# fjdf/slaMEM

Hardware: AMD Instinct MI355X
Metric: MEMs/sec (and queries/sec) on 100 Mbp ref x 10 M 150 bp queries, l=20 (higher is better)
Workload: dtype u32; 1 GPU; synthetic 100000000 bp reference (splitmix64 seed 42) x 10000000 reads/GPU of 150 bp, 2% substitutions, 50% reverse-complemented, -b -l 20; ref_len=100000000, reads_total=10000000, read_len=150, min_len=20, both_strands=True, parallelism=query shards x1, one GPU, no replication

## Files before the change

slamem_amd/csrc/mem_search.hip:

```cpp
#include "common.h"
#include "prims.h"

#include <atomic>
#include <type_traits>
#include <new>
#include <stdlib.h>
#include <string.h>

namespace slamem {

struct Blk {
    uint4 a;
    uint4 b;
    uint4 c;
    uint4 d;
};

__device__ __forceinline__ uint64_t u64_of(uint32_t lo, uint32_t hi) { return ((uint64_t)hi << 32) | lo; }

__device__ __forceinline__ Blk load_blk(const FMBlock* __restrict__ fm, uint32_t bi) {
    const uint4* p = reinterpret_cast<const uint4*>(fm + bi);
    Blk k;
    k.a = p[0]; k.b = p[1]; k.c = p[2]; k.d = p[3];
    return k;
// ... 82 lines not shown
__device__ __forceinline__ int parent_from(const uint4& rt, const uint4& rb, uint32_t& top, uint32_t& bot) {
    uint32_t a = rt.x, b = rb.z;
    uint32_t d = a > b ? a : b;
    if (d == 0u) return -1;
    if (a == d) top = rt.y;
    if (b == d) bot = rb.w - 1u;
    return (int)(d - 1u);
}

__device__ __forceinline__ int parent(const IndexView& ix, uint32_t& top, uint32_t& bot) {
    const uint4* R = reinterpret_cast<const uint4*>(ix.rec);
    uint4 rt = R[top], rb = R[bot];
    return parent_from(rt, rb, top, bot);
}

__device__ __forceinline__ uint32_t ascii_code_q(uint32_t ch) {
    uint32_t x = ch & 0xDFu;
    return x == 'A' ? 2u : x == 'C' ? 3u : x == 'G' ? 4u : x == 'T' ? 5u : 1u;
}

struct SearchArgs {
    IndexView ix;
    const uint64_t* qwords;
    const uint64_t* offsets;
    uint32_t num_queries;
    uint32_t strands;
    uint32_t min_len;
    int32_t pad0;
    uint32_t pad1;
    uint32_t pad;
    uint64_t capacity;
    unsigned long long* total;
    RawKey* raw_key;
    slamem_mem* raw_mem;
    uint32_t* block_counts;
    struct RawRow* inline_rows;
    uint64_t inline_stride;
    const struct ItemDesc* items;
    uint64_t num_items;
    uint8_t* item_attempt;
    const uint8_t* item_alive;
    const uint32_t* work_ids;
    const uint32_t* work_count;
    unsigned long long* stats;
    uint64_t query_words;
    const uint64_t* pq;
    uint64_t* pq_out;
    uint32_t implicit_items;
    uint32_t* seed_left_ids;
    unsigned int* seed_left_count;
    unsigned int* seed_long_flag;
    unsigned int* seed_wide;
    uint32_t seed_step;
    const uint64_t* item_pk;
    unsigned int* work_cursor;
    int32_t direct_min_depth;
    uint32_t use_jump;
    uint32_t pad2;
    uint32_t skip_w;
    const uint64_t* pq2;
    uint64_t* pq2_out;
    uint8_t* item_flags;
    uint32_t skip_s1;
    uint32_t pad4;
    const struct SliceState* slice_state;
    const uint32_t* item_block;
    struct OutCtx {
        struct RawRow* inline_rows;
        uint64_t inline_stride;
        RawKey* raw_key;
        slamem_mem* raw_mem;
        unsigned long long* total;
        uint64_t capacity;
        uint32_t* block_counts;
        uint8_t* item_attempt;
    } prev;
    struct DeferCtx {
        struct JobRec* queue;
        unsigned int* njobs;
        uint32_t* pool;
        unsigned int* pool_next;
        uint32_t pool_cap;
        uint32_t queue_cap;
        uint32_t epoch;
        uint32_t* raw_seg;
        uint2* list;
        unsigned int* nlist;
        uint8_t* inline_valid;
    } defer;
    const struct CarryRec* carry_in;
    const unsigned int* carry_in_count;
    struct CarryRec* carry_out;
    unsigned int* carry_out_count;
};

struct RawRow { uint32_t row, pos, len; };
constexpr uint32_t kInlineMems = 4;
constexpr uint32_t kFetch = 64;

constexpr uint32_t kSliceLen = 4096;
static_assert(kSliceLen == kSearchSliceLen, "stream.hip tells the slice count of a batch from this length");
constexpr uint32_t kWarmUp = 1024;
constexpr uint32_t kMaxAttempt = 7;
struct __attribute__((aligned(16))) ItemDesc {
    uint64_t base;
    uint32_t len;
// ... 1819 lines not shown
                const uint32_t my_wave = threadIdx.x >> 6;
                res = 0;
#pragma unroll 1
                for (uint32_t first = 0; first < 4u; first += per_part) {
                    lo = span_lo(first, per_part);
                    hi = span_hi(first, per_part);
                    if (hi <= lo) continue;
                    __syncthreads();
                    pack_span(lo, (uint32_t)(hi - lo));
                    if (my_wave >= first && my_wave < first + per_part)
                        res = prefilter_item_packed<kStats>(A, d, s_pk, s_nm, (uint32_t)(d.base - (lo << 4)), n_probe);
                }
            } else {
                res = prefilter_item<kStats>(A, d, n_probe, n_qload);
            }
        }
    } else {
        res = prefilter_item<kStats>(A, d, n_probe, n_qload);
    }
    if (live) alive[g] = res;
    if (kStats) {
        stat_flush<kStats>(A.stats + SC_PF_PROBES, n_probe);
        stat_flush<kStats>(A.stats + SC_PF_QUERY_LOADS, n_qload);
        stat_flush<kStats>(A.stats + SC_PF_ITEMS, live ? 1u : 0u);
    }
}

__global__ void __launch_bounds__(256) k_prefilter_list(SearchArgs A, const uint32_t* __restrict__ list, const uint32_t* __restrict__ list_count,
                                                        uint8_t* __restrict__ alive) {
    const uint32_t count = *list_count;
    for (uint32_t i = blockIdx.x * blockDim.x + threadIdx.x; i < count; i += gridDim.x * blockDim.x) {
        const uint32_t g = list[i];
        const ItemDesc d = item_of(A, g);
        uint32_t n_probe = 0, n_qload = 0;
        if (!prefilter_item<false>(A, d, n_probe, n_qload)) alive[g] = 0;
    }
}

#ifndef SLAMEM_SEED_READS
#define SLAMEM_SEED_READS 21
#endif
constexpr uint32_t kSeedReads = SLAMEM_SEED_READS, kSeedReadsMid = 16, kSeedReadsLong = 16;
constexpr uint32_t kSeedMaxLen = 192;
constexpr uint32_t kSeedMaxLenMid = 256;
constexpr uint32_t kSeedMaxLenLong = 384;
#ifndef SLAMEM_SEED_JOBS
#define SLAMEM_SEED_JOBS 16
#endif
constexpr uint32_t kSeedJobs = SLAMEM_SEED_JOBS;
#ifndef SLAMEM_SEED_MEMS
#define SLAMEM_SEED_MEMS 12
#endif
constexpr uint32_t kSeedMems = SLAMEM_SEED_MEMS;
constexpr uint32_t kSigLetters = 12, kSigMask = (1u << kSigLetters) - 1u, kSigKnown = 1u << 24;

template <uint32_t NW, uint32_t R>
struct SeedWave {
    static constexpr uint32_t kJobs = kSeedJobs * R * NW / 3u, kMems = kSeedMems * R * NW / 3u;
    uint64_t pl[R][2][2][NW + 1];
    uint32_t len[R];
    uint32_t nwin[R];
    union {
        uint4 raw[R * NW * 4 + 1];
        struct {
            uint32_t job_p[kJobs], job_x[kJobs];
            uint32_t mem_key[kMems], mem_ref[kMems];
            uint32_t mem_sig[kMems];
        };
    };
    uint32_t bad[R];
    uint64_t pn[R][NW + 1];
    uint32_t hasn;
    unsigned long long expl[R];
    union {
        uint16_t ring[128];
        unsigned long long smask[2 * R];
    };
    uint32_t flags;
    uint32_t pad[3];
};

__device__ __forceinline__ void wave_sync() {
    __builtin_amdgcn_fence(__ATOMIC_RELEASE, "wavefront");
    __builtin_amdgcn_wave_barrier();
    __builtin_amdgcn_fence(__ATOMIC_ACQUIRE, "wavefront");
}
__device__ __forceinline__ uint64_t funnel64(uint64_t lo, uint64_t hi, uint32_t sh) { return (lo >> sh) | ((hi << 1) << (63u - sh)); }
__device__ __forceinline__ uint64_t bits_below(int x) {
    const int c = x < 0 ? 0 : x > 64 ? 64 : x;
    return c == 0 ? 0ull : (~0ull >> (64 - c));
}
__device__ __forceinline__ uint64_t bits_range(int lo, int hi) { return bits_below(hi) & ~bits_below(lo); }
__device__ __forceinline__ uint32_t sel4(const uint4& v, uint32_t a) {
    const uint32_t lo = (a & 1u) ? v.y : v.x, hi = (a & 1u) ? v.w : v.z;
    return (a & 2u) ? hi : lo;
}
__device__ __forceinline__ uint32_t sel12(const uint4& b0, const uint4& b1, const uint4& b2, uint32_t e) {
    const uint32_t a = e & 3u, x0 = sel4(b0, a), x1 = sel4(b1, a), x2 = sel4(b2, a);
    return e < 4u ? x0 : e < 8u ? x1 : x2;
}
__device__ __forceinline__ uint32_t byte_tops(uint32_t m) {
    const uint32_t y = m >> 7;
    return (y | (y >> 7) | (y >> 14) | (y >> 21)) & 0xFu;
}

#ifndef SLAMEM_SEED_WAVES
#define SLAMEM_SEED_WAVES 1
#endif
template <bool kStats, uint32_t NW, uint32_t R>
__global__ void __launch_bounds__(256, SLAMEM_SEED_WAVES) k_seed_mems(SearchArgs A, uint8_t* __restrict__ alive) {
    constexpr uint32_t kMaxLen = 64u * NW;
    static_assert(R <= 32u && R * NW <= 128u, "a flag word holds a bit per read; the planes step runs in at most two passes");
    __shared__ SeedWave<NW, R> lds[4];
    const IndexView& ix = A.ix;
    const uint32_t lane = threadIdx.x & 63u, wv = threadIdx.x >> 6;
    SeedWave<NW, R>& S = lds[wv];
    const uint32_t strands = A.strands, k = ix.seed_k, L = A.min_len, s = L - k + 1u;
    const uint32_t kmask = (1u << k) - 1u;
    const uint64_t r0 = ((uint64_t)blockIdx.x * 4u + wv) * R;
    if (r0 >= (uint64_t)A.num_queries) return;
    const uint32_t nr = (uint64_t)A.num_queries - r0 < R ? (uint32_t)((uint64_t)A.num_queries - r0) : R;
    const unsigned long long below = (1ull << lane) - 1ull;
    const int64_t ulast = (int64_t)text_units(ix.n) - 1;
    uint32_t n_win = 0, n_cmp = 0, n_nm = 0, n_mem = 0;

    const uint64_t off = lane <= nr ? A.offsets[r0 + lane] : 0ull;
    constexpr uint32_t kRawChunks = R * NW * 4u + 1u, kSpecIters = (kRawChunks + 63u) / 64u;
#ifndef SLAMEM_SEED_NO_SPEC
    constexpr bool kSpec = kSpecIters <= 5u;
#else
    constexpr bool kSpec = false;
#endif
    uint4 sv[kSpec ? kSpecIters : 1u];
    uint64_t g0 = 0, len0 = 0;
    bool spec = false;
    if (kSpec) {
        const uint64_t o0 = A.offsets[0], o1 = A.offsets[1], o_end = A.offsets[A.num_queries];
        len0 = o1 - o0;
        g0 = o0 + r0 * len0;
        const uint64_t g1 = g0 + (uint64_t)nr * len0;
        spec = len0 != 0ull && len0 <= (uint64_t)kMaxLen && g1 <= o_end;
        const uint32_t gn = spec ? (uint32_t)(((g1 - 1u) >> 4) - (g0 >> 4) + 1u) : 0u;
        const uint4* src = reinterpret_cast<const uint4*>(A.qwords) + (g0 >> 4);
#pragma unroll
        for (uint32_t j = 0; j < kSpecIters; j++) {
            const uint32_t c = lane + 64u * j;
            sv[j] = c < gn ? src[c] : make_uint4(0, 0, 0, 0);
        }
    }
    const uint64_t offn = __shfl_down(off, 1);
    if (kSpec) spec = spec && __ballot(lane <= nr && off != g0 + (uint64_t)lane * len0) == 0ull;
    uint32_t len = 0, nwin = 0;
    bool left = false;
    if (lane < nr) {
        const uint64_t l64 = offn - off;
        if (l64 > kSliceLen) atomicOr(A.seed_long_flag, 1u);
// ... 75 lines not shown
                const uint32_t tt = B2 & ~B1, good = (B0 ^ tt) & ~((B4 ^ tt) | B3 | B7) & B6;
                bad |= ~good & M;
                const uint32_t X = ((B1 ^ B2) & M) | ((B2 & M) << 4);
                const uint32_t G = (X | (X >> 7) | (X >> 14) | (X >> 21)) & 0xFFu;
                if (t < 8u) { p0lo |= (G & 0xFu) << (4u * t); p1lo |= (G >> 4) << (4u * t); }
                else { p0hi |= (G & 0xFu) << (4u * (t - 8u)); p1hi |= (G >> 4) << (4u * (t - 8u)); }
            }
            S.pl[i][0][0][j] = u64_of(p0lo, p0hi);
            S.pl[i][0][1][j] = u64_of(p1lo, p1hi);
            uint32_t nlo = 0, nhi = 0;
            if (bad && text_pure) {
#pragma unroll
                for (uint32_t t = 0; t < 16u; t++) {
                    const uint32_t d = __builtin_amdgcn_alignbyte(w[t + 1u], w[t], sh8);
                    const uint32_t nb = nv > 4u * t ? (nv - 4u * t < 4u ? nv - 4u * t : 4u) : 0u;
                    const uint32_t M = nb >= 4u ? 0x01010101u : (0x01010101u & ((1u << (8u * nb)) - 1u));
                    const uint32_t B0 = d, B1 = d >> 1, B2 = d >> 2, B3 = d >> 3, B4 = d >> 4, B6 = d >> 6, B7 = d >> 7;
                    const uint32_t tt = B2 & ~B1, X = ~((B0 ^ tt) & ~((B4 ^ tt) | B3 | B7) & B6) & M;
                    const uint32_t G = (X | (X >> 7) | (X >> 14) | (X >> 21)) & 0xFu;
                    if (t < 8u) nlo |= G << (4u * t); else nhi |= G << (4u * (t - 8u));
                }
                S.hasn = 1u;
            } else if (bad) S.bad[i] = 1u;
            S.pn[i][j] = u64_of(nlo, nhi);
        } else if (on) {
            S.pl[i][0][0][j] = 0ull; S.pl[i][0][1][j] = 0ull; S.pn[i][j] = 0ull;
        }
        if (on && j == 0u) { S.pl[i][0][0][NW] = 0ull; S.pl[i][0][1][NW] = 0ull; S.pl[i][1][0][NW] = 0ull; S.pl[i][1][1][NW] = 0ull; S.pn[i][NW] = 0ull; }
    }
    wave_sync();
    for (uint32_t pb = 0; pb < nr * NW; pb += 64u) {
        const uint32_t pp = pb + lane, i = pp / NW, w = pp % NW;
        const bool on = pp < nr * NW;
        const uint32_t Li = __shfl(plen, (int)(on ? i : 0u));
        if (on) {
            const uint32_t sh = kMaxLen - Li, q = sh >> 6, r = sh & 63u;
#pragma unroll
            for (uint32_t pl = 0; pl < 2u; pl++) {
                const uint64_t* f = S.pl[i][0][pl];
                const uint64_t lo = w + q < NW ? __brevll(f[NW - 1u - (w + q)]) : 0ull, hi = w + q + 1u < NW ? __brevll(f[NW - 2u - (w + q)]) : 0ull;
                S.pl[i][1][pl][w] = Li ? ~funnel64(lo, hi, r) & bits_range(0, (int)Li - 64 * (int)w) : 0ull;
            }
        }
    }
    {
        const bool isbad = lane < nr && plen != 0u && S.bad[lane] != 0u;
        wflags |= (uint32_t)__ballot(isbad);
        if (isbad) nwin = 0;
        if (lane < nr) { S.len[lane] = nwin ? len : 0u; S.nwin[lane] = nwin; }
    }
    if (lane == 0u)
        for (uint32_t i = nr; i < R; i++) { S.len[i] = 0u; S.nwin[i] = 0u; }
    wave_sync();
    const uint32_t mfit = k / s > 6u ? 6u : k / s;
    const uint32_t mstep = A.seed_step ? A.seed_step : mfit >= 3u ? mfit : s <= 12u ? 2u : 1u;

    const bool wave_hasn = __builtin_amdgcn_readfirstlane((int)S.hasn) != 0;
    uint32_t lg_slots = 0;
    {
        const uint32_t nwl = lane < nr ? S.nwin[lane] : 0u;
#pragma unroll
        for (uint32_t t = 1, lg = 1; t <= 32u; t <<= 1, lg++)
            if (__ballot(nwl > t) != 0ull) lg_slots = lg;
    }
    if (lane < R) S.expl[lane] = 0ull;
    uint32_t njobs = 0, nmems = 0;

    auto search = [&](auto with_n) {
    constexpr bool hasn = decltype(with_n)::value;
    auto trip = [&](uint32_t ent, bool act, uint32_t step) {
        const uint32_t rs = ent >> 8, wi = ent & 0xFFu;
        const uint32_t Lr = act ? S.len[rs] : 0u;
        const uint32_t o = wi * s;
        uint32_t want = 0, pal = 0;
        uint4 b0 = make_uint4(0, 0, 0, 0), b1 = b0, b2 = b0, b3 = b0;
        if (hasn && act) {
            const uint64_t* PN = S.pn[rs];
            if (((uint32_t)funnel64(PN[o >> 6], PN[(o >> 6) + 1u], o & 63u) & kmask) != 0u) act = false;
        }
        if (act) {
            const uint32_t q = o >> 6, sh = o & 63u;
            const uint64_t* P0 = S.pl[rs][0][0];
            const uint64_t* P1 = S.pl[rs][0][1];
            const uint32_t f0 = (uint32_t)funnel64(P0[q], P0[q + 1u], sh) & kmask, f1 = (uint32_t)funnel64(P1[q], P1[q + 1u], sh) & kmask;
            uint32_t bucket, tagbits, orient;
            seed_place(f0, f1, k, ix.seed_log2, bucket, tagbits, orient, pal);
            want = tagbits | (orient << 7);
            const uint4* B = reinterpret_cast<const uint4*>(ix.seed + bucket);
            b0 = B[0]; b1 = B[1]; b2 = B[2]; b3 = B[3];
        }
        if (kStats) n_win += (uint32_t)__popcll(__ballot(act));
        const uint32_t wbytes = want * 0x01010101u;
        const uint32_t x0 = b3.x ^ wbytes, x1 = b3.y ^ wbytes, x2 = b3.z ^ wbytes;
        const uint32_t m0 = ~((x0 & 0x7F7F7F7Fu) + 0x7F7F7F7Fu) & 0x80808080u, m1 = ~((x1 & 0x7F7F7F7Fu) + 0x7F7F7F7Fu) & 0x80808080u,
                       m2 = ~((x2 & 0x7F7F7F7Fu) + 0x7F7F7F7Fu) & 0x80808080u;
        const uint32_t count = b3.w;
        uint32_t hits = byte_tops(m0) | (byte_tops(m1) << 4) | (byte_tops(m2) << 8);
        const uint32_t rev = byte_tops(x0 & 0x80808080u) | (byte_tops(x1 & 0x80808080u) << 4) | (byte_tops(x2 & 0x80808080u) << 8);
        hits &= count >= kSeedSlots ? 0xFFFu : (1u << count) - 1u;
        if (strands == 1u && step == 1u) hits &= ~rev;
        if (!act) hits = 0;
        const uint32_t xn = act && (count & kSeedSpilled) ? (count >> 24) & 0x1Fu : 0u, xo = (count & 0xFFFFFFu) << 2;
        if (act && count > kSeedSlots && !(count & kSeedSpilled)) {
            atomicOr(&S.flags, 1u << rs);
            if (kStats) atomicAdd(A.stats + SC_SEED_WHY + 1u, 1ull);
            hits = 0;
        }
        const bool both = pal != 0u && strands == 2u;
        if (kStats && both && hits) atomicAdd(A.stats + SC_SEED_WHY + 2u, 1ull);
        const uint32_t e1 = hits ? (uint32_t)__ffs((int)hits) - 1u : 0u;
        const uint32_t p1 = sel12(b0, b1, b2, e1);
        const uint32_t st1 = (rev >> e1) & 1u;
        const uint32_t dist = step * s;
        uint32_t pn = 0, pp1 = 0, ps1 = 0;
        if (dist <= k) {
            pp1 = __shfl_up(p1, 1);
            ps1 = __shfl_up(hits ? st1 : 2u, 1);
            const uint32_t pent = __shfl_up(act ? ent : 0xFFFFFFFFu, 1);
            pn = (lane == 0u || wi < step || pent != ent - step || ps1 == 2u) ? 0u : 1u;
        }
        const uint32_t njobs0 = njobs;
        auto push = [&](bool hv, uint32_t p, uint32_t st) {
            const uint32_t w = st ? p + dist : p - dist;
            const bool job = hv && !(pn && pp1 == w && ps1 == st);
            const unsigned long long qb = __ballot(job);
            const uint32_t at = njobs + (uint32_t)__popcll(qb & below);
            if (job && at < SeedWave<NW, R>::kJobs) {
                S.job_p[at] = p;
                S.job_x[at] = (st ? Lr - k - o : o) | (st << 15) | (rs << 16);
            }
            njobs += (uint32_t)__popcll(qb);
        };
        uint32_t rem = hits;
        for (uint32_t it = 0; __ballot(rem != 0u) != 0ull; it++) {
            const bool hv = rem != 0u;
            const uint32_t e = it == 0u ? e1 : hv ? (uint32_t)__ffs((int)rem) - 1u : 0u;
            rem &= rem - 1u;
            const uint32_t p = it == 0u ? p1 : sel12(b0, b1, b2, e);
            push(hv, p, (rev >> e) & 1u);
            if (__ballot(hv && both) != 0ull) push(hv && both, p, 1u);
        }
        for (uint32_t e0 = 0; __ballot(e0 < xn) != 0ull; e0 += 4u) {
            const bool on = e0 < xn;
            uint4 v0 = make_uint4(0, 0, 0, 0), v1 = v0;
            if (on) {
                const uint4* P = reinterpret_cast<const uint4*>(ix.spill + xo + e0);
                v0 = P[0]; v1 = P[1];
            }
#pragma unroll
            for (uint32_t q = 0; q < 4u; q++) {
                const uint32_t p = q == 0u ? v0.x : q == 1u ? v0.z : q == 2u ? v1.x : v1.z;
                const uint32_t d = ((q == 0u ? v0.y : q == 1u ? v0.w : q == 2u ? v1.y : v1.w) ^ want) & 0xFFu;
                const uint32_t st = d >> 7;
                const bool hv = on && e0 + q < xn && (d & 0x7Fu) == 0u && !(strands == 1u && st && step == 1u);
                if (__ballot(hv) == 0ull) continue;
                push(hv, p, st);
                if (__ballot(hv && both) != 0ull) push(hv && both, p, 1u);
            }
        }
        if (njobs > SeedWave<NW, R>::kJobs) {
            if (act) atomicOr(&S.flags, 1u << rs);
            if (kStats && lane == 0u) atomicAdd(A.stats + SC_SEED_WHY + 3u, 1ull);
            njobs = njobs0;
        }
    };
    auto lookups = [&](uint32_t round) {
        const uint32_t step = round == 0u ? mstep : 1u;
        uint32_t cnt = 0;
        const uint32_t per = 64u >> lg_slots, wi = lane & ((1u << lg_slots) - 1u);
        const uint32_t wmod = wi - mstep * ((wi * (65536u / mstep + 1u)) >> 16);
        for (uint32_t r = 0;; r += per) {
            if (r < nr) {
                const uint32_t rr = r + (lane >> lg_slots);
                const uint32_t nw = (rr >= nr || ((S.flags >> rr) & 1u)) ? 0u : S.nwin[rr];
                const bool pred = wi < nw && (round == 0u ? wmod == 0u : wmod != 0u && ((S.expl[rr] >> wi) & 1ull) == 0ull);
                const unsigned long long pm = __ballot(pred);
                if (pred) S.ring[cnt + (uint32_t)__popcll(pm & below)] = (uint16_t)((rr << 8) | wi);
                cnt += (uint32_t)__popcll(pm);
            }
            const bool last = r >= nr;
            if (cnt >= 64u || (last && cnt != 0u)) {
                wave_sync();
                const bool act = lane < cnt;
                const uint32_t ent = act ? S.ring[lane] : 0u;
                const uint32_t over = lane + 64u < cnt ? S.ring[lane + 64u] : 0u;
                wave_sync();
                if (lane + 64u < cnt) S.ring[lane] = (uint16_t)over;
                cnt = cnt > 64u ? cnt - 64u : 0u;
                trip(ent, act, step);
            }
            if (last) break;
        }
        wave_sync();
    };

    auto compares = [&](uint32_t round) {
        const bool mark = round == 0u && mstep > 1u;
        const uint32_t ms = mstep * s;
        const uint32_t gone = S.flags;
        for (uint32_t jb = 0; jb < njobs; jb += 64u) {
            const bool listed = jb + lane < njobs;
            const uint32_t p = listed ? S.job_p[jb + lane] : 0u, xx = listed ? S.job_x[jb + lane] : 0u;
            const uint32_t os = xx & 0x7FFFu, st = (xx >> 15) & 1u, jr = xx >> 16;
            const bool has = listed && ((gone >> jr) & 1u) == 0u;
            const uint32_t Lj = S.len[jr];
            const int64_t d = (int64_t)p - (int64_t)os;
            const int64_t u0 = d >> 6;
            const uint32_t sh = (uint32_t)(d & 63);
            bool is_mem = false;
            uint32_t key = 0, ref = 0, sig = 0;
            if (has) {
                constexpr int NU = (int)NW + 1;
                int64_t ui[NU];
#pragma unroll
                for (int i = 0; i < NU; i++) { const int64_t u = u0 + i; ui[i] = u < 0 ? 0 : u > ulast ? ulast : u; }
                const uint4* T = reinterpret_cast<const uint4*>(ix.tpl);
                uint4 tu[NU], tx[NU];
#pragma unroll
                for (int i = 0; i < NU; i++) { tu[i] = T[2 * ui[i]]; tx[i] = T[2 * ui[i] + 1]; }
                uint64_t uq[NU], nu[NU];
                uint32_t anyn = 0;
#pragma unroll
                for (int i = 0; i < NU; i++) { nu[i] = u64_of(tx[i].x, tx[i].y); uq[i] = u64_of(tx[i].z, tx[i].w); anyn |= (tx[i].x | tx[i].y); }
                if (kStats && anyn) n_nm++;
                const uint64_t* R0 = S.pl[jr][st][0];
                const uint64_t* R1 = S.pl[jr][st][1];
                uint64_t mm[NW];
#pragma unroll
                for (int w = 0; w < (int)NW; w++)
                    mm[w] = (funnel64(u64_of(tu[w].x, tu[w].y), u64_of(tu[w + 1].x, tu[w + 1].y), sh) ^ R0[w]) |
                            (funnel64(u64_of(tu[w].z, tu[w].w), u64_of(tu[w + 1].z, tu[w + 1].w), sh) ^ R1[w]) | funnel64(nu[w], nu[w + 1], sh);
                if (hasn) {
                    const uint64_t* PN = S.pn[jr];
                    if (st == 0u) {
#pragma unroll
                        for (int w = 0; w < (int)NW; w++) mm[w] |= PN[w];
                    } else {
                        const uint32_t shn = kMaxLen - Lj, qn = shn >> 6, rn = shn & 63u;
#pragma unroll
                        for (int w = 0; w < (int)NW; w++) {
                            const uint32_t x = (uint32_t)w + qn;
                            const uint64_t lo64 = x < NW ? __brevll(PN[NW - 1u - x]) : 0ull, hi64 = x + 1u < NW ? __brevll(PN[NW - 2u - x]) : 0ull;
                            mm[w] |= funnel64(lo64, hi64, rn);
                        }
                    }
                }
                const int lo = d < 0 ? (int)(-d) : 0;
                const int64_t room = (int64_t)ix.n - d;
                const int hi = room < (int64_t)Lj ? (int)room : (int)Lj;
#pragma unroll
                for (int w = 0; w < (int)NW; w++) mm[w] |= ~bits_range(lo - 64 * w, hi - 64 * w);
                uint32_t a = 0, b = kMaxLen;
                bool broken = false;
#pragma unroll
                for (int w = 0; w < (int)NW; w++) {
                    const uint64_t lw = mm[w] & bits_range(0, (int)os - 64 * w);
                    if (lw) a = 64u * w + 64u - (uint32_t)__clzll((long long)lw);
                    if (mm[w] & bits_range((int)os - 64 * w, (int)(os + k) - 64 * w)) broken = true;
                }
#pragma unroll
                for (int w = (int)NW - 1; w >= 0; w--) {
                    const uint64_t hw = mm[w] & ~bits_range(0, (int)(os + k) - 64 * w);
                    if (hw) b = 64u * w + (uint32_t)__ffsll((unsigned long long)hw) - 1u;
                }
                const uint32_t af = st ? Lj - b : a, bf = st ? Lj - a : b, of = st ? Lj - k - os : os;
                bool owner;
                if (round == 0u) owner = !(of >= ms && of - ms >= af);
                else {
                    const uint32_t oa = (af + ms - 1u) / ms * ms;
                    owner = !(mstep > 1u && oa + k <= bf) && !(of >= s && of - s >= af);
                }
                if (broken) {
                    atomicOr(&S.flags, 1u << jr);
                    if (kStats) atomicAdd(A.stats + SC_SEED_WHY + 4u, 1ull);
                }
                else if (owner && b - a >= L && (strands == 2u || st == 0u)) {
                    is_mem = true; key = (a << 16) | (b - a); ref = (uint32_t)(d + (int64_t)a);
                    if (!anyn && b + kSigLetters <= kMaxLen && d + (int64_t)b + (int64_t)kSigLetters <= (int64_t)ix.n) {
                        const uint32_t wb = b >> 6, sb = b & 63u;
                        uint64_t l0 = 0, h0 = 0, l1 = 0, h1 = 0;
#pragma unroll
                        for (int w = 0; w < (int)NW; w++) {
                            const uint64_t t0 = funnel64(u64_of(tu[w].x, tu[w].y), u64_of(tu[w + 1].x, tu[w + 1].y), sh);
                            const uint64_t t1 = funnel64(u64_of(tu[w].z, tu[w].w), u64_of(tu[w + 1].z, tu[w + 1].w), sh);
                            if ((uint32_t)w == wb) { l0 = t0; l1 = t1; }
                            if ((uint32_t)w == wb + 1u) { h0 = t0; h1 = t1; }
                        }
                        sig = kSigKnown | ((uint32_t)funnel64(l0, h0, sb) & kSigMask) | (((uint32_t)funnel64(l1, h1, sb) & kSigMask) << kSigLetters);
                    }
                }
                if (mark && !broken && bf >= af + k) {
                    uint64_t uqs[NW];
#pragma unroll
                    for (int w = 0; w < (int)NW; w++) uqs[w] = funnel64(uq[w], uq[w + 1], sh);
                    unsigned long long done = 0ull;
                    for (uint32_t wi = (af + s - 1u) / s, wl = (bf - k) / s; wi <= wl; wi++) {
                        const uint32_t x = st ? Lj - k - wi * s : wi * s;
                        uint64_t word = 0ull;
#pragma unroll
                        for (int w = 0; w < (int)NW; w++) word = (x >> 6) == (uint32_t)w ? uqs[w] : word;
                        if ((word >> (x & 63u)) & 1ull) done |= 1ull << wi;
                    }
                    if (done) atomicOr(&S.expl[jr], done);
                }
            }
            if (kStats) {
                const uint32_t nh = (uint32_t)__popcll(__ballot(has));
                n_cmp += nh;
                if (mark && lane == 0u) atomicAdd(A.stats + SC_SEED_ONCE, (unsigned long long)nh);
            }
            const unsigned long long mb = __ballot(is_mem);
            if (is_mem) {
                const uint32_t at = nmems + (uint32_t)__popcll(mb & below);
                if (at < SeedWave<NW, R>::kMems) { S.mem_key[at] = key; S.mem_ref[at] = ref; S.mem_sig[at] = sig | ((2u * jr + st) << 25); }
                else { atomicOr(&S.flags, 1u << jr); if (kStats) atomicAdd(A.stats + SC_SEED_WHY + 5u, 1ull); }
            }
            nmems += (uint32_t)__popcll(mb);
        }
        wave_sync();
    };

    for (uint32_t round = 0; round < (mstep > 1u ? 2u : 1u); round++) {
        njobs = 0;
        lookups(round);
        compares(round);
    }
    };
    if (wave_hasn) search(std::true_type{}); else search(std::false_type{});
    {
        if (nmems > SeedWave<NW, R>::kMems) nmems = SeedWave<NW, R>::kMems;

        const uint32_t g0 = (uint32_t)(r0 * strands);
        auto rank_of = [&](uint32_t mi, uint32_t key, uint32_t g, uint32_t& rank, uint32_t& cnt, bool& tie) {
            rank = 0; cnt = 0; tie = false;
            for (uint32_t t2 = 0; t2 < nmems; t2++) {
                const uint32_t kk = S.mem_key[t2], gg = S.mem_sig[t2] >> 25;
                const bool same = gg == g;
                cnt += same ? 1u : 0u;
                rank += (same && kk > key) ? 1u : 0u;
                tie = tie || (same && kk == key && t2 != mi);
            }
        };
        auto tie_rank = [&](uint32_t mi, uint32_t key, uint32_t myref, uint32_t g, uint32_t sig, uint32_t& rank) -> bool {
            const uint32_t a = key >> 16, b = a + (key & 0xFFFFu);
            bool child = false;
            for (uint32_t t2 = 0; t2 < nmems; t2++) {
                const uint32_t kk = S.mem_key[t2], a2 = kk >> 16, b2 = a2 + (kk & 0xFFFFu);
                child = child || ((S.mem_sig[t2] >> 25) == g && kk != key && a2 <= a && b2 > b);
            }
            const uint32_t jr = g >> 1, st = g & 1u;
            uint32_t qb = 0;
            if (child) qb = (uint32_t)((S.pl[jr][st][0][b >> 6] >> (b & 63u)) & 1ull) | ((uint32_t)((S.pl[jr][st][1][b >> 6] >> (b & 63u)) & 1ull) << 1);
            auto letter = [&](uint32_t sg, uint32_t t) { return ((sg >> t) & 1u) | (((sg >> (t + kSigLetters)) & 1u) << 1); };
            const bool rows = ix.prec != nullptr;
            const uint32_t my_side = child && letter(sig, 0u) > qb ? 1u : 0u;
            bool bad = (sig & kSigKnown) == 0u && (child || !rows);
            for (uint32_t t2 = 0; t2 < nmems; t2++) {
                const uint32_t so = S.mem_sig[t2];
                if (t2 == mi || (so >> 25) != g || S.mem_key[t2] != key) continue;
                const bool known = (so & sig & kSigKnown) != 0u;
                if (!known && (child || !rows)) { bad = true; continue; }
                const uint32_t o_side = child && letter(so, 0u) > qb ? 1u : 0u;
                bool before;
                if (o_side != my_side) before = o_side == 0u;
                else {
                    const uint32_t x = sig ^ so, diff = known ? (x | (x >> kSigLetters)) & kSigMask : 0u;
                    bool smaller;
                    if (diff != 0u) {
                        const uint32_t t = (uint32_t)__ffs((int)diff) - 1u;
                        smaller = letter(so, t) < letter(sig, t);
                    } else if (rows) smaller = ix.prec[S.mem_ref[t2]].row < ix.prec[myref].row;
                    else { bad = true; continue; }
                    before = my_side == 0u ? smaller : !smaller;
                }
                rank += before ? 1u : 0u;
// ... 559 lines not shown
        STEP(hipMemsetAsync(d_pq, 0, 16, stream), "memset");
        A.pq = d_pq;
        A.pq_out = d_pq;
        A.item_pk = seed_path ? nullptr : d_itempk;
        static const int env_depth = [] { const char* v = getenv("SLAMEM_DIRECT_DEPTH"); return v ? atoi(v) : 0; }();
        int lg = 0;
        for (uint64_t v = idx->hdr.n; v > 1; v >>= 2) lg++;
        A.direct_min_depth = (idx->view.tgrp && depth_class((int)min_len) >= 1u) ? lg + 3 : -1;
        if (env_depth > 0 && A.direct_min_depth >= 0) A.direct_min_depth = env_depth;
        if (env_depth < 0) A.direct_min_depth = -1;
        static const bool env_jump = [] { const char* v = getenv("SLAMEM_KJUMP_USE"); return !(v && atoi(v) == 0); }();
        A.use_jump = env_jump ? 1u : 0u;
        {
            static const bool env_skip = [] { const char* v = getenv("SLAMEM_SKIP"); return v && atoi(v) != 0; }();
            const uint32_t kd = idx->view.kbits ? idx->view.kbits_k : 0u;
            A.skip_w = 0;
            if (env_skip && kd && min_len >= kd && min_len >= 9u && min_len < 0x10000u && A.direct_min_depth >= 0) {
                const uint32_t s1 = min_len - kd + 1u;
                const uint32_t nprobes = (kd - 1u + s1 - 1u) / s1 + 1u;
                if (nprobes <= 4u && depth_class((int)min_len - 1) >= 1u) {
                    A.skip_w = min_len - 1u;
                    A.skip_s1 = s1;
                    A.pq2 = reinterpret_cast<const uint64_t*>(ws + w.off_pq2);
                    A.pq2_out = reinterpret_cast<uint64_t*>(ws + w.off_pq2);
                    A.item_flags = reinterpret_cast<uint8_t*>(ws + w.off_itemflags);
                }
            }
        }
    }
    return SLAMEM_OK;
}

int SearchJob::prep(hipStream_t stream) {
    SLAMEM_HIP(hipSetDevice(idx->device));
    char* ws = static_cast<char*>(workspace_dev);
    unsigned long long* d_total = reinterpret_cast<unsigned long long*>(ws + w.off_total);
    uint32_t* d_counts = reinterpret_cast<uint32_t*>(ws + w.off_counts);
    prefiltered = false; timed_k8 = false; launched = true; seeded = false; rawkey_marked = false;
    (void)hipEventRecord(ev[0], stream);
    if (nitems && (match_type != 1 || mam_v3)) {
        static const bool use_filter = [] { const char* v = getenv("SLAMEM_KFILTER"); return !(v && atoi(v) == 0); }();
        seeded = seed_path;
        if (seeded) {
            uint8_t* d_alive = reinterpret_cast<uint8_t*>(ws + w.off_alive);
            if (mems_capacity && !A.skip_w && !want_stats && enum_chunks()) {
                STEP(hipMemsetAsync(ws + w.off_rawkey, 0xFF, mems_capacity * sizeof(RawKey), stream), "memset");
                rawkey_marked = true;
            }
            STEP(hipMemsetAsync(d_counts, 0, nitems * 4, stream), "memset");
            STEP(hipMemsetAsync(A.item_attempt, 0, nitems, stream), "memset");
            {
                const char* v = getenv("SLAMEM_SEED_STEP");
                A.seed_step = v && atoi(v) >= 1 && atoi(v) <= 6 ? (uint32_t)atoi(v) : 0u;
            }
            uint32_t* d_ids = reinterpret_cast<uint32_t*>(ws + w.off_workids);
            uint32_t* d_nwork = reinterpret_cast<uint32_t*>(d_total) + 8;
            A.seed_left_ids = d_ids;
            A.seed_left_count = d_nwork;
            A.seed_long_flag = reinterpret_cast<unsigned int*>(d_total) + 3;
            A.seed_wide = reinterpret_cast<unsigned int*>(d_total) + 4;
            seed_words_avg = query_bytes > (uint64_t)num_queries * kSeedMaxLenMid ? 6u : query_bytes > (uint64_t)num_queries * kSeedMaxLen ? 4u : 3u;
            const uint32_t hint = __atomic_load_n(&idx->seed_words_hint, __ATOMIC_RELAXED);
            seed_words = seed_words_avg > hint ? seed_words_avg : hint;
            const bool mid_reads = seed_words == 4u, long_reads = seed_words == 6u;
            const dim3 gs(grid_for((uint64_t)num_queries, 4 * (long_reads ? kSeedReadsLong : mid_reads ? kSeedReadsMid : kSeedReads)));
            if (long_reads) {
                if (want_stats) hipLaunchKernelGGL((k_seed_mems<true, 6, kSeedReadsLong>), gs, dim3(256), 0, stream, A, d_alive);
                else hipLaunchKernelGGL((k_seed_mems<false, 6, kSeedReadsLong>), gs, dim3(256), 0, stream, A, d_alive);
            } else if (mid_reads) {
                if (want_stats) hipLaunchKernelGGL((k_seed_mems<true, 4, kSeedReadsMid>), gs, dim3(256), 0, stream, A, d_alive);
                else hipLaunchKernelGGL((k_seed_mems<false, 4, kSeedReadsMid>), gs, dim3(256), 0, stream, A, d_alive);
            } else {
                if (want_stats) hipLaunchKernelGGL((k_seed_mems<true, 3, kSeedReads>), gs, dim3(256), 0, stream, A, d_alive);
                else hipLaunchKernelGGL((k_seed_mems<false, 3, kSeedReads>), gs, dim3(256), 0, stream, A, d_alive);
            }
            STEP(hipGetLastError(), "k_seed_mems");
            (void)hipEventRecord(ev[3], stream);
            prefiltered = true;
            A.item_alive = d_alive;
            A.work_ids = d_ids;
            A.work_count = d_nwork;
            if (use_filter && idx->view.kfilter && min_len >= idx->view.kfilter_k) {
                hipLaunchKernelGGL(k_prefilter_list, dim3(512), dim3(256), 0, stream, A, (const uint32_t*)d_ids, (const uint32_t*)d_nwork, d_alive);
                STEP(hipGetLastError(), "k_prefilter_list");
            }
        } else if (use_filter && idx->view.kfilter && min_len >= idx->view.kfilter_k) {
            uint8_t* d_alive = reinterpret_cast<uint8_t*>(ws + w.off_alive);
            if (want_stats) hipLaunchKernelGGL(k_prefilter<true>, dim3(grid_for(nitems)), dim3(256), 0, stream, A, d_alive);
            else hipLaunchKernelGGL(k_prefilter<false>, dim3(grid_for(nitems)), dim3(256), 0, stream, A, d_alive);
            STEP(hipGetLastError(), "k_prefilter");
            (void)hipEventRecord(ev[3], stream);
            prefiltered = true;
            A.item_alive = d_alive;
            STEP(hipMemsetAsync(d_counts, 0, nitems * 4, stream), "memset");
            STEP(hipMemsetAsync(A.item_attempt, 0, nitems, stream), "memset");
            uint32_t* d_ids = reinterpret_cast<uint32_t*>(ws + w.off_workids);
            uint32_t* d_nwork = reinterpret_cast<uint32_t*>(d_total) + 8;
            size_t need2 = w.select_bytes;
            STEP(select_indices_u32(ws + w.off_select, need2, d_alive, d_ids, d_nwork, nitems, stream), "select");
            A.work_ids = d_ids;
            A.work_count = d_nwork;
        }
        if (A.item_flags) STEP(hipMemsetAsync(A.item_flags, 0, nitems, stream), "memset");
        if (nitems != num_blocks) {
            static const uint32_t env_warm = [] { const char* v = getenv("SLAMEM_SLICE_WARMUP"); return v && atoi(v) > 0 ? (uint32_t)atoi(v) : kWarmUp; }();
            SliceState* d_states = reinterpret_cast<SliceState*>(ws + w.off_slicestate);
// ... 484 lines not shown
```

Measured before the change: 4.480 billion MEMs/s.

## Seed MEM search from a few sparse windows, then fill uncovered windows

Replaces the fixed-stride first round of seed lookups with a sparse first round that probes only a few evenly spaced windows per read (default 3, settable through SLAMEM_SEED_FIRST). It then marks, per query position, which k-mers are already covered by extended agreement runs, so the second round skips covered windows. A memo of the last diagonal found also suppresses duplicate jobs. The aim is fewer hash lookups and fewer reference compares per read, paid for with bit-parallel agreement masks, multi-MEM enumeration per job, and a larger shared-memory explored array, all of which add compute and register pressure.

```diff
diff --git a/slamem_amd/csrc/mem_search.hip b/slamem_amd/csrc/mem_search.hip
--- a/slamem_amd/csrc/mem_search.hip
+++ b/slamem_amd/csrc/mem_search.hip
@@ -158,6 +158,7 @@
     unsigned int* seed_long_flag;
     unsigned int* seed_wide;
     uint32_t seed_step;
+    uint32_t seed_first;
     const uint64_t* item_pk;
     unsigned int* work_cursor;
     int32_t direct_min_depth;
@@ -2083,6 +2084,11 @@
 #define SLAMEM_SEED_MEMS 12
 #endif
 constexpr uint32_t kSeedMems = SLAMEM_SEED_MEMS;
+#ifndef SLAMEM_SEED_FIRST
+#define SLAMEM_SEED_FIRST 3
+#endif
+constexpr uint32_t kSeedFirst = SLAMEM_SEED_FIRST;
+static_assert(kSeedFirst >= 1u && kSeedFirst <= 8u, "SLAMEM_SEED_FIRST: 1..8");
 constexpr uint32_t kSigLetters = 12, kSigMask = (1u << kSigLetters) - 1u, kSigKnown = 1u << 24;
 
 template <uint32_t NW, uint32_t R>
@@ -2099,10 +2105,13 @@
             uint32_t mem_sig[kMems];
         };
     };
-    uint32_t bad[R];
+    union {
+        uint32_t bad[R];
+        uint32_t adia[R];
+    };
     uint64_t pn[R][NW + 1];
     uint32_t hasn;
-    unsigned long long expl[R];
+    unsigned long long expl[R][NW];
     union {
         uint16_t ring[128];
         unsigned long long smask[2 * R];
@@ -2133,6 +2142,36 @@
 __device__ __forceinline__ uint32_t byte_tops(uint32_t m) {
     const uint32_t y = m >> 7;
     return (y | (y >> 7) | (y >> 14) | (y >> 21)) & 0xFu;
+}
+
+template <uint32_t NW>
+__device__ __forceinline__ void and_shr(uint64_t (&v)[NW], uint32_t c) {
+#pragma unroll
+    for (uint32_t w = 0; w < NW; w++) v[w] &= funnel64(v[w], w + 1u < NW ? v[w + 1u] : 0ull, c);
+}
+template <uint32_t NW>
+__device__ __forceinline__ void agree_from(const uint64_t (&mm)[NW], uint32_t k, uint64_t (&a)[NW]) {
+#pragma unroll
+    for (uint32_t w = 0; w < NW; w++) a[w] = ~mm[w];
+    uint32_t span = 1;
+    for (; 2u * span <= k; span *= 2u) and_shr<NW>(a, span);
+    if (span < k) and_shr<NW>(a, k - span);
+}
+template <uint32_t NW>
+__device__ __forceinline__ void to_forward(uint64_t (&v)[NW], uint32_t sh) {
+    uint64_t r[NW], p[NW];
+#pragma unroll
+    for (uint32_t w = 0; w < NW; w++) r[w] = __brevll(v[NW - 1u - w]);
+    const uint32_t q = sh >> 6, rr = sh & 63u;
+#pragma unroll
+    for (uint32_t i = 0; i < NW; i++) p[i] = funnel64(r[i], i + 1u < NW ? r[i + 1u] : 0ull, rr);
+#pragma unroll
+    for (uint32_t w = 0; w < NW; w++) {
+        uint64_t x = 0ull;
+#pragma unroll
+        for (uint32_t i = w; i < NW; i++) x = i == w + q ? p[i] : x;
+        v[w] = x;
+    }
 }
 
 #ifndef SLAMEM_SEED_WAVES
@@ -2314,26 +2353,45 @@
     if (lane == 0u)
         for (uint32_t i = nr; i < R; i++) { S.len[i] = 0u; S.nwin[i] = 0u; }
     wave_sync();
-    const uint32_t mfit = k / s > 6u ? 6u : k / s;
-    const uint32_t mstep = A.seed_step ? A.seed_step : mfit >= 3u ? mfit : s <= 12u ? 2u : 1u;
+    const bool sparse = A.seed_step == 0u;
+    const uint32_t mstep = sparse ? 1u : A.seed_step, nfirst = sparse ? (s <= 12u ? A.seed_first : 64u) : mstep > 1u ? 1u : 64u;
 
     const bool wave_hasn = __builtin_amdgcn_readfirstlane((int)S.hasn) != 0;
     uint32_t lg_slots = 0;
+    uint32_t nwmax = 0;
     {
         const uint32_t nwl = lane < nr ? S.nwin[lane] : 0u;
 #pragma unroll
         for (uint32_t t = 1, lg = 1; t <= 32u; t <<= 1, lg++)
             if (__ballot(nwl > t) != 0ull) lg_slots = lg;
-    }
-    if (lane < R) S.expl[lane] = 0ull;
+#pragma unroll
+        for (uint32_t bit = 64u; bit != 0u; bit >>= 1)
+            if (__ballot(nwl >= (nwmax | bit)) != 0ull) nwmax |= bit;
+    }
+    unsigned long long fwu = bits_below((int)nwmax);
+    if (mstep > 1u) {
+        unsigned long long m = 0ull;
+        for (uint32_t w = 0; w < 64u; w += mstep) m |= 1ull << w;
+        fwu &= m;
+    } else if (sparse && nwmax > nfirst) {
+        const uint32_t frcp = 65536u / (2u * nfirst) + 1u;
+        fwu = 0ull;
+        for (uint32_t j = 0; j < nfirst; j++) fwu |= 1ull << ((((2u * j + 1u) * nwmax) * frcp) >> 16);
+    }
+    auto has_b = [&](uint32_t nw) { return (bits_below((int)nw) & ~fwu) != 0ull; };
+    const bool two = __ballot(lane < nr && has_b(S.nwin[lane])) != 0ull;
+    for (uint32_t i = lane; i < R * NW; i += 64u) (&S.expl[0][0])[i] = 0ull;
+    if (lane < R) S.adia[lane] = 0xFFFFFFFFu;
+    const bool memo = (uint64_t)ix.n + 2u * kMaxLen < 0x7FFFFFFFull;
     uint32_t njobs = 0, nmems = 0;
 
     auto search = [&](auto with_n) {
     constexpr bool hasn = decltype(with_n)::value;
-    auto trip = [&](uint32_t ent, bool act, uint32_t step) {
+    auto trip = [&](uint32_t ent, bool act, uint32_t round) {
         const uint32_t rs = ent >> 8, wi = ent & 0xFFu;
         const uint32_t Lr = act ? S.len[rs] : 0u;
         const uint32_t o = wi * s;
+        const bool marks = round == 0u && act && has_b(S.nwin[rs]);
         uint32_t want = 0, pal = 0;
         uint4 b0 = make_uint4(0, 0, 0, 0), b1 = b0, b2 = b0, b3 = b0;
         if (hasn && act) {
@@ -2360,7 +2418,7 @@
         uint32_t hits = byte_tops(m0) | (byte_tops(m1) << 4) | (byte_tops(m2) << 8);
         const uint32_t rev = byte_tops(x0 & 0x80808080u) | (byte_tops(x1 & 0x80808080u) << 4) | (byte_tops(x2 & 0x80808080u) << 8);
         hits &= count >= kSeedSlots ? 0xFFFu : (1u << count) - 1u;
-        if (strands == 1u && step == 1u) hits &= ~rev;
+        if (strands == 1u && !marks) hits &= ~rev;
         if (!act) hits = 0;
         const uint32_t xn = act && (count & kSeedSpilled) ? (count >> 24) & 0x1Fu : 0u, xo = (count & 0xFFFFFFu) << 2;
         if (act && count > kSeedSlots && !(count & kSeedSpilled)) {
@@ -2373,18 +2431,15 @@
         const uint32_t e1 = hits ? (uint32_t)__ffs((int)hits) - 1u : 0u;
         const uint32_t p1 = sel12(b0, b1, b2, e1);
         const uint32_t st1 = (rev >> e1) & 1u;
-        const uint32_t dist = step * s;
-        uint32_t pn = 0, pp1 = 0, ps1 = 0;
-        if (dist <= k) {
-            pp1 = __shfl_up(p1, 1);
-            ps1 = __shfl_up(hits ? st1 : 2u, 1);
-            const uint32_t pent = __shfl_up(act ? ent : 0xFFFFFFFFu, 1);
-            pn = (lane == 0u || wi < step || pent != ent - step || ps1 == 2u) ? 0u : 1u;
-        }
+        const uint32_t ps1 = __shfl_up(hits ? st1 : 2u, 1), pp1 = __shfl_up(p1, 1), pent = __shfl_up(act ? ent : 0xFFFFFFFFu, 1);
+        const uint32_t dist1 = (wi - (pent & 0xFFu)) * s;
+        const uint32_t e1s = lane != 0u && (pent >> 8) == rs && (two || dist1 <= k) ? ps1 : 2u, e1p = ps1 ? pp1 - dist1 : pp1 + dist1;
+        const bool use_memo = round != 0u && memo && act;
+        const uint32_t adia = use_memo ? S.adia[rs] : 0xFFFFFFFFu;
         const uint32_t njobs0 = njobs;
         auto push = [&](bool hv, uint32_t p, uint32_t st) {
-            const uint32_t w = st ? p + dist : p - dist;
-            const bool job = hv && !(pn && pp1 == w && ps1 == st);
+            const uint32_t dc = (p - (st ? Lr - k - o : o) + kMaxLen) | (st << 31);
+            const bool job = hv && !(e1s == st && e1p == p) && !(use_memo && dc == adia);
             const unsigned long long qb = __ballot(job);
             const uint32_t at = njobs + (uint32_t)__popcll(qb & below);
             if (job && at < SeedWave<NW, R>::kJobs) {
@@ -2414,7 +2469,7 @@
                 const uint32_t p = q == 0u ? v0.x : q == 1u ? v0.z : q == 2u ? v1.x : v1.z;
                 const uint32_t d = ((q == 0u ? v0.y : q == 1u ? v0.w : q == 2u ? v1.y : v1.w) ^ want) & 0xFFu;
                 const uint32_t st = d >> 7;
-                const bool hv = on && e0 + q < xn && (d & 0x7Fu) == 0u && !(strands == 1u && st && step == 1u);
+                const bool hv = on && e0 + q < xn && (d & 0x7Fu) == 0u && !(strands == 1u && st && !marks);
                 if (__ballot(hv) == 0ull) continue;
                 push(hv, p, st);
                 if (__ballot(hv && both) != 0ull) push(hv && both, p, 1u);
@@ -2427,15 +2482,14 @@
         }
     };
     auto lookups = [&](uint32_t round) {
-        const uint32_t step = round == 0u ? mstep : 1u;
         uint32_t cnt = 0;
         const uint32_t per = 64u >> lg_slots, wi = lane & ((1u << lg_slots) - 1u);
-        const uint32_t wmod = wi - mstep * ((wi * (65536u / mstep + 1u)) >> 16);
         for (uint32_t r = 0;; r += per) {
             if (r < nr) {
                 const uint32_t rr = r + (lane >> lg_slots);
                 const uint32_t nw = (rr >= nr || ((S.flags >> rr) & 1u)) ? 0u : S.nwin[rr];
-                const bool pred = wi < nw && (round == 0u ? wmod == 0u : wmod != 0u && ((S.expl[rr] >> wi) & 1ull) == 0ull);
+                const bool fa = ((fwu >> wi) & 1ull) != 0ull;
+                const bool pred = wi < nw && (round == 0u ? fa : !fa && ((S.expl[rr][(wi * s) >> 6] >> ((wi * s) & 63u)) & 1ull) == 0ull);
                 const unsigned long long pm = __ballot(pred);
                 if (pred) S.ring[cnt + (uint32_t)__popcll(pm & below)] = (uint16_t)((rr << 8) | wi);
                 cnt += (uint32_t)__popcll(pm);
@@ -2449,7 +2503,7 @@
                 wave_sync();
                 if (lane + 64u < cnt) S.ring[lane] = (uint16_t)over;
                 cnt = cnt > 64u ? cnt - 64u : 0u;
-                trip(ent, act, step);
+                trip(ent, act, round);
             }
             if (last) break;
         }
@@ -2457,9 +2511,24 @@
     };
 
     auto compares = [&](uint32_t round) {
-        const bool mark = round == 0u && mstep > 1u;
-        const uint32_t ms = mstep * s;
+        const bool mark = round == 0u && two;
         const uint32_t gone = S.flags;
+        uint64_t wall[NW], fa[NW];
+        {
+            uint32_t o1 = 0;
+#pragma unroll
+            for (uint32_t w = 0; w < NW; w++) {
+                uint64_t x1 = 0ull;
+                for (; two && o1 < 64u * w + 64u; o1 += s) x1 |= 1ull << (o1 - 64u * w);
+                wall[w] = x1;
+                fa[w] = 0ull;
+            }
+            for (unsigned long long m = two ? fwu : 0ull; m != 0ull; m &= m - 1ull) {
+                const uint32_t oj = (uint32_t)(__ffsll(m) - 1) * s;
+#pragma unroll
+                for (uint32_t w = 0; w < NW; w++) fa[w] |= (oj >> 6) == w ? 1ull << (oj & 63u) : 0ull;
+            }
+        }
         for (uint32_t jb = 0; jb < njobs; jb += 64u) {
             const bool listed = jb + lane < njobs;
             const uint32_t p = listed ? S.job_p[jb + lane] : 0u, xx = listed ? S.job_x[jb + lane] : 0u;
@@ -2469,8 +2538,13 @@
             const int64_t d = (int64_t)p - (int64_t)os;
             const int64_t u0 = d >> 6;
             const uint32_t sh = (uint32_t)(d & 63);
-            bool is_mem = false;
-            uint32_t key = 0, ref = 0, sig = 0;
+            uint64_t run[NW];
+            uint64_t mm[NW];
+            uint64_t tt0[NW], tt1[NW];
+            uint32_t anyn = 0;
+            bool report = false;
+#pragma unroll
+            for (int w = 0; w < (int)NW; w++) run[w] = 0ull;
             if (has) {
                 constexpr int NU = (int)NW + 1;
                 int64_t ui[NU];
@@ -2481,17 +2555,17 @@
 #pragma unroll
                 for (int i = 0; i < NU; i++) { tu[i] = T[2 * ui[i]]; tx[i] = T[2 * ui[i] + 1]; }
                 uint64_t uq[NU], nu[NU];
-                uint32_t anyn = 0;
 #pragma unroll
                 for (int i = 0; i < NU; i++) { nu[i] = u64_of(tx[i].x, tx[i].y); uq[i] = u64_of(tx[i].z, tx[i].w); anyn |= (tx[i].x | tx[i].y); }
                 if (kStats && anyn) n_nm++;
                 const uint64_t* R0 = S.pl[jr][st][0];
                 const uint64_t* R1 = S.pl[jr][st][1];
-                uint64_t mm[NW];
-#pragma unroll
-                for (int w = 0; w < (int)NW; w++)
-                    mm[w] = (funnel64(u64_of(tu[w].x, tu[w].y), u64_of(tu[w + 1].x, tu[w + 1].y), sh) ^ R0[w]) |
-                            (funnel64(u64_of(tu[w].z, tu[w].w), u64_of(tu[w + 1].z, tu[w + 1].w), sh) ^ R1[w]) | funnel64(nu[w], nu[w + 1], sh);
+#pragma unroll
+                for (int w = 0; w < (int)NW; w++) {
+                    tt0[w] = funnel64(u64_of(tu[w].x, tu[w].y), u64_of(tu[w + 1].x, tu[w + 1].y), sh);
+                    tt1[w] = funnel64(u64_of(tu[w].z, tu[w].w), u64_of(tu[w + 1].z, tu[w + 1].w), sh);
+                    mm[w] = (tt0[w] ^ R0[w]) | (tt1[w] ^ R1[w]) | funnel64(nu[w], nu[w + 1], sh);
+                }
                 if (hasn) {
                     const uint64_t* PN = S.pn[jr];
                     if (st == 0u) {
@@ -2512,58 +2586,60 @@
                 const int hi = room < (int64_t)Lj ? (int)room : (int)Lj;
 #pragma unroll
                 for (int w = 0; w < (int)NW; w++) mm[w] |= ~bits_range(lo - 64 * w, hi - 64 * w);
-                uint32_t a = 0, b = kMaxLen;
-                bool broken = false;
-#pragma unroll
-                for (int w = 0; w < (int)NW; w++) {
-                    const uint64_t lw = mm[w] & bits_range(0, (int)os - 64 * w);
-                    if (lw) a = 64u * w + 64u - (uint32_t)__clzll((long long)lw);
-                    if (mm[w] & bits_range((int)os - 64 * w, (int)(os + k) - 64 * w)) broken = true;
-                }
-#pragma unroll
-                for (int w = (int)NW - 1; w >= 0; w--) {
-                    const uint64_t hw = mm[w] & ~bits_range(0, (int)(os + k) - 64 * w);
-                    if (hw) b = 64u * w + (uint32_t)__ffsll((unsigned long long)hw) - 1u;
-                }
-                const uint32_t af = st ? Lj - b : a, bf = st ? Lj - a : b, of = st ? Lj - k - os : os;
-                bool owner;
-                if (round == 0u) owner = !(of >= ms && of - ms >= af);
-                else {
-                    const uint32_t oa = (af + ms - 1u) / ms * ms;
-                    owner = !(mstep > 1u && oa + k <= bf) && !(of >= s && of - s >= af);
+                const uint32_t of = st ? Lj - k - os : os;
+                bool broken = false, owner;
+                uint64_t ak[NW];
+                if (!two) {
+                    uint32_t a = 0, b = kMaxLen;
+#pragma unroll
+                    for (int w = 0; w < (int)NW; w++) {
+                        const uint64_t lw = mm[w] & bits_range(0, (int)os - 64 * w);
+                        if (lw) a = 64u * w + 64u - (uint32_t)__clzll((long long)lw);
+                        if (mm[w] & bits_range((int)os - 64 * w, (int)(os + k) - 64 * w)) broken = true;
+                    }
+#pragma unroll
+                    for (int w = (int)NW - 1; w >= 0; w--) {
+                        const uint64_t hw = mm[w] & ~bits_range(0, (int)(os + k) - 64 * w);
+                        if (hw) b = 64u * w + (uint32_t)__ffsll((unsigned long long)hw) - 1u;
+                    }
+                    const uint32_t af0 = st ? Lj - b : a;
+                    owner = !(of >= s && of - s >= af0);
+#pragma unroll
+                    for (int w = 0; w < (int)NW; w++) ak[w] = b - a >= L && (a >> 6) == (uint32_t)w ? 1ull << (a & 63u) : 0ull;
+                } else {
+                    agree_from<NW>(mm, k, ak);
+                    broken = true;
+#pragma unroll
+                    for (int w = 0; w < (int)NW; w++)
+                        if ((os >> 6) == (uint32_t)w) broken = ((ak[w] >> (os & 63u)) & 1ull) == 0ull;
+                    uint64_t af[NW];
+#pragma unroll
+                    for (int w = 0; w < (int)NW; w++) af[w] = ak[w];
+                    if (st) to_forward<NW>(af, kMaxLen - 1u - (Lj - k));
+                    uint64_t other = 0ull;
+#pragma unroll
+                    for (int w = 0; w < (int)NW; w++) {
+                        const uint64_t before = bits_range(0, (int)of - 64 * w);
+                        other |= af[w] & (round == 0u ? fa[w] & before : fa[w] | (wall[w] & before));
+                    }
+                    owner = other == 0ull;
                 }
                 if (broken) {
                     atomicOr(&S.flags, 1u << jr);
                     if (kStats) atomicAdd(A.stats + SC_SEED_WHY + 4u, 1ull);
-                }
-                else if (owner && b - a >= L && (strands == 2u || st == 0u)) {
-                    is_mem = true; key = (a << 16) | (b - a); ref = (uint32_t)(d + (int64_t)a);
-                    if (!anyn && b + kSigLetters <= kMaxLen && d + (int64_t)b + (int64_t)kSigLetters <= (int64_t)ix.n) {
-                        const uint32_t wb = b >> 6, sb = b & 63u;
-                        uint64_t l0 = 0, h0 = 0, l1 = 0, h1 = 0;
-#pragma unroll
-                        for (int w = 0; w < (int)NW; w++) {
-                            const uint64_t t0 = funnel64(u64_of(tu[w].x, tu[w].y), u64_of(tu[w + 1].x, tu[w + 1].y), sh);
-                            const uint64_t t1 = funnel64(u64_of(tu[w].z, tu[w].w), u64_of(tu[w + 1].z, tu[w + 1].w), sh);
-                            if ((uint32_t)w == wb) { l0 = t0; l1 = t1; }
-                            if ((uint32_t)w == wb + 1u) { h0 = t0; h1 = t1; }
-                        }
-                        sig = kSigKnown | ((uint32_t)funnel64(l0, h0, sb) & kSigMask) | (((uint32_t)funnel64(l1, h1, sb) & kSigMask) << kSigLetters);
+                } else if (owner) {
+                    report = strands == 2u || st == 0u;
+#pragma unroll
+                    for (int w = 0; w < (int)NW; w++) run[w] = report ? ak[w] : 0ull;
+                    if (mark && has_b(S.nwin[jr])) {
+                        uint64_t done[NW];
+#pragma unroll
+                        for (int w = 0; w < (int)NW; w++) done[w] = ak[w] & funnel64(uq[w], uq[w + 1], sh);
+                        if (st) to_forward<NW>(done, kMaxLen - 1u - (Lj - k));
+#pragma unroll
+                        for (int w = 0; w < (int)NW; w++)
+                            if (done[w]) atomicOr(&S.expl[jr][w], (unsigned long long)done[w]);
                     }
-                }
-                if (mark && !broken && bf >= af + k) {
-                    uint64_t uqs[NW];
-#pragma unroll
-                    for (int w = 0; w < (int)NW; w++) uqs[w] = funnel64(uq[w], uq[w + 1], sh);
-                    unsigned long long done = 0ull;
-                    for (uint32_t wi = (af + s - 1u) / s, wl = (bf - k) / s; wi <= wl; wi++) {
-                        const uint32_t x = st ? Lj - k - wi * s : wi * s;
-                        uint64_t word = 0ull;
-#pragma unroll
-                        for (int w = 0; w < (int)NW; w++) word = (x >> 6) == (uint32_t)w ? uqs[w] : word;
-                        if ((word >> (x & 63u)) & 1ull) done |= 1ull << wi;
-                    }
-                    if (done) atomicOr(&S.expl[jr], done);
                 }
             }
             if (kStats) {
@@ -2571,18 +2647,53 @@
                 n_cmp += nh;
                 if (mark && lane == 0u) atomicAdd(A.stats + SC_SEED_ONCE, (unsigned long long)nh);
             }
-            const unsigned long long mb = __ballot(is_mem);
-            if (is_mem) {
-                const uint32_t at = nmems + (uint32_t)__popcll(mb & below);
-                if (at < SeedWave<NW, R>::kMems) { S.mem_key[at] = key; S.mem_ref[at] = ref; S.mem_sig[at] = sig | ((2u * jr + st) << 25); }
-                else { atomicOr(&S.flags, 1u << jr); if (kStats) atomicAdd(A.stats + SC_SEED_WHY + 5u, 1ull); }
-            }
-            nmems += (uint32_t)__popcll(mb);
+            bool more = false;
+#pragma unroll
+            for (int w = 0; w < (int)NW; w++) more = more || run[w] != 0ull;
+            while (__ballot(more) != 0ull) {
+                bool is_mem = false;
+                uint32_t key = 0, ref = 0, sig = 0;
+                if (more) {
+                    uint32_t a = kMaxLen, b = kMaxLen;
+#pragma unroll
+                    for (int w = (int)NW - 1; w >= 0; w--)
+                        if (run[w]) a = 64u * w + (uint32_t)__ffsll((unsigned long long)run[w]) - 1u;
+#pragma unroll
+                    for (int w = (int)NW - 1; w >= 0; w--) {
+                        const uint64_t hw = mm[w] & ~bits_below((int)a - 64 * w);
+                        if (hw) b = 64u * w + (uint32_t)__ffsll((unsigned long long)hw) - 1u;
+                    }
+                    more = false;
+#pragma unroll
+                    for (int w = 0; w < (int)NW; w++) { run[w] &= ~bits_below((int)b - 64 * w); more = more || run[w] != 0ull; }
+                    if (b - a >= L) {
+                        is_mem = true; key = (a << 16) | (b - a); ref = (uint32_t)(d + (int64_t)a);
+                        if (mark && memo) S.adia[jr] = (uint32_t)(d + (int64_t)kMaxLen) | (st << 31);
+                        if (!anyn && b + kSigLetters <= kMaxLen && d + (int64_t)b + (int64_t)kSigLetters <= (int64_t)ix.n) {
+                            const uint32_t wb = b >> 6, sb = b & 63u;
+                            uint64_t l0 = 0, h0 = 0, l1 = 0, h1 = 0;
+#pragma unroll
+                            for (int w = 0; w < (int)NW; w++) {
+                                if ((uint32_t)w == wb) { l0 = tt0[w]; l1 = tt1[w]; }
+                                if ((uint32_t)w == wb + 1u) { h0 = tt0[w]; h1 = tt1[w]; }
+                            }
+                            sig = kSigKnown | ((uint32_t)funnel64(l0, h0, sb) & kSigMask) | (((uint32_t)funnel64(l1, h1, sb) & kSigMask) << kSigLetters);
+                        }
+                    }
+                }
+                const unsigned long long mb = __ballot(is_mem);
+                if (is_mem) {
+                    const uint32_t at = nmems + (uint32_t)__popcll(mb & below);
+                    if (at < SeedWave<NW, R>::kMems) { S.mem_key[at] = key; S.mem_ref[at] = ref; S.mem_sig[at] = sig | ((2u * jr + st) << 25); }
+                    else { atomicOr(&S.flags, 1u << jr); if (kStats) atomicAdd(A.stats + SC_SEED_WHY + 5u, 1ull); }
+                }
+                nmems += (uint32_t)__popcll(mb);
+            }
         }
         wave_sync();
     };
 
-    for (uint32_t round = 0; round < (mstep > 1u ? 2u : 1u); round++) {
+    for (uint32_t round = 0; round < (two ? 2u : 1u); round++) {
         njobs = 0;
         lookups(round);
         compares(round);
@@ -3248,6 +3359,8 @@
             {
                 const char* v = getenv("SLAMEM_SEED_STEP");
                 A.seed_step = v && atoi(v) >= 1 && atoi(v) <= 6 ? (uint32_t)atoi(v) : 0u;
+                const char* f = getenv("SLAMEM_SEED_FIRST");
+                A.seed_first = f && atoi(f) >= 1 && atoi(f) <= 8 ? (uint32_t)atoi(f) : kSeedFirst;
             }
             uint32_t* d_ids = reinterpret_cast<uint32_t*>(ws + w.off_workids);
             uint32_t* d_nwork = reinterpret_cast<uint32_t*>(d_total) + 8;
```

Measured after the change: 5.057 billion MEMs/s, median of 6. 12.9% higher.
